# emmanuel-marty/zultra

Hardware: NVIDIA B200
Metric: input MB/s (zultra compression hot path, byte-identical to CPU zultra) (higher is better)
Workload: dtype u8

## Files before the change

### zultra_b200/csrc/zb_pipeline.h

```cpp
#ifndef ZB_PIPELINE_H
#define ZB_PIPELINE_H
#include "zb_rt.h"
#include <vector>
#include <algorithm>
#ifndef ZB_EMU
#include <cuda_pipeline.h>
#endif

#ifndef ZB_CG
#define ZB_CG 1024
#endif
#ifndef ZB_CP
#define ZB_CP 1024
#endif
#define ZB_CD 2048
#define ZB_WU 384
#define ZB_TOKI 256
#define ZB_NH 320
#define ZB_MAXSB 64
#define ZB_MAXNODES 64
#define ZB_MF_TILE_MAX 16384

struct ZbWinDesc {
   uint32_t in_off;
   uint32_t hist;
   uint32_t len;
   uint32_t stream;
   uint32_t last;
   uint32_t pad[3];
};

struct ZbNode {
   uint32_t win, depth;
   uint32_t ts, te;
   uint32_t ps, pe;
   uint32_t t0, nchk;
   uint32_t chk_base;
   int32_t total_cost;
   int32_t best_delta; uint32_t best_tok;
   uint32_t pad[4];
};

struct ZbSub {
   uint32_t win, idx_in_win;
   uint32_t ps, pe;
   uint32_t ts, te;
   int32_t is_dyn, static_cost, dynamic_cost;
   uint32_t dchunk_base, ndchunk;
   uint32_t pchunk_base, npchunk;
   int32_t mask, nl, no, ncl;
   int32_t hdr_bits;
   int32_t body_bits;
   int32_t stored;
   int32_t final_bit;
   uint64_t bit_off;
   int32_t ub_hit; int32_t pad;
};

struct ZbSubTabs {
   int lcnt[ZB_NLIT], ocnt[ZB_NOFF];
   int llen[ZB_NLIT], olen[ZB_NOFF];
   uint16_t lcode[ZB_NLIT], ocode[ZB_NOFF];
   int cllen[ZB_NCL]; uint16_t clcode[ZB_NCL];
   alignas(16) uint8_t cl[ZB_NLIT + ZB_NOFF]; int mask_cost[20];
   ZbCostTab cost;
};

struct ZbStreamOut {
   uint64_t out_word_off;
   uint64_t in_bits;
   uint64_t total_bits;
   uint32_t first_win, nwin;
   uint32_t err, pad;
};

ZB_HD void zb_tok_count(const uint8_t *T, uint32_t p, uint32_t len, uint32_t off, int *lc, int *oc, int sign) {
   if (len >= ZB_MIN_MATCH) { lc[zb_len_sym(len - ZB_MIN_MATCH)] += sign; oc[zb_off_sym(off)] += sign; }
   else lc[T[p]] += sign;
}

ZB_HD int zb_warmup_len(int WU, int reach) {
   const int margin = WU > ZB_MAX_MATCH ? WU - ZB_MAX_MATCH : 0;
   const int w = reach + margin;
   return w < WU ? w : WU;
}

template <class T> struct ZbBuf {
   T *p = 0; size_t cap = 0;
   void need(size_t n) { if (n > cap) { zb_dev_free(p); size_t c = n + n / 8 + 64; p = (T *)zb_dev_alloc(c * sizeof(T)); cap = p ? c : 0; } }
   void release() { zb_dev_free(p); p = 0; cap = 0; }
};

struct ZbHostBuf {
   uint8_t *p = 0; size_t cap = 0;
   void need(size_t n) { if (n > cap) { zb_host_free(p); size_t c = n + n / 8 + 4096; p = (uint8_t *)zb_host_alloc(c); cap = p ? c : 0; } }
   void release() { zb_host_free(p); p = 0; cap = 0; }
};

#ifndef ZB_EMU
#include <thread>
struct ZbStager {
   enum { LANES = 4, PIECE = 4 << 20 };
   uint8_t *buf = 0; cudaStream_t st[LANES]; cudaEvent_t ev[LANES][2]; bool ready = false;
   bool init() {
      if (ready) return true;
      if (cudaHostAlloc((void **)&buf, (size_t)LANES * 2 * PIECE, cudaHostAllocDefault) != cudaSuccess) { cudaGetLastError(); buf = 0; return false; }
      for (int l = 0; l < LANES; l++) { cudaStreamCreateWithFlags(&st[l], cudaStreamNonBlocking); cudaEventCreateWithFlags(&ev[l][0], cudaEventDisableTiming); cudaEventCreateWithFlags(&ev[l][1], cudaEventDisableTiming); }
      ready = true;
      return true;
   }
   void release() { if (!ready) return; for (int l = 0; l < LANES; l++) { cudaStreamDestroy(st[l]); cudaEventDestroy(ev[l][0]); cudaEventDestroy(ev[l][1]); } cudaFreeHost(buf); buf = 0; ready = false; }
   static bool pageable(const void *p) {
      cudaPointerAttributes a;
      if (cudaPointerGetAttributes(&a, p) != cudaSuccess) { cudaGetLastError(); return true; }
      return a.type == cudaMemoryTypeUnregistered;
   }
   bool copy(int dir, void *dev, void *host, size_t n, int device) {
      if (!init()) return false;
      bool ok[LANES];
      auto lane = [&](int l) {
         ok[l] = true;
         if (cudaSetDevice(device) != cudaSuccess) { ok[l] = false; return; }
         const size_t per = ((n + LANES - 1) / LANES + 255) & ~(size_t)255, lo = std::min(n, (size_t)l * per), hi = std::min(n, lo + per);
         uint8_t *b[2] = {buf + (size_t)(2 * l) * PIECE, buf + (size_t)(2 * l + 1) * PIECE};
         size_t pend_off[2] = {0, 0}, pend_len[2] = {0, 0};
         int k = 0;
         for (size_t off = lo; off < hi; off += PIECE, k ^= 1) {
            const size_t len = std::min((size_t)PIECE, hi - off);
            if (dir == 0) {
               if (cudaEventSynchronize(ev[l][k]) != cudaSuccess) ok[l] = false;
               memcpy(b[k], (const uint8_t *)host + off, len);
               if (cudaMemcpyAsync((uint8_t *)dev + off, b[k], len, cudaMemcpyHostToDevice, st[l]) != cudaSuccess) ok[l] = false;
               cudaEventRecord(ev[l][k], st[l]);
            } else {
               if (pend_len[k]) { if (cudaEventSynchronize(ev[l][k]) != cudaSuccess) ok[l] = false; memcpy((uint8_t *)host + pend_off[k], b[k], pend_len[k]); }
               if (cudaMemcpyAsync(b[k], (const uint8_t *)dev + off, len, cudaMemcpyDeviceToHost, st[l]) != cudaSuccess) ok[l] = false;
               cudaEventRecord(ev[l][k], st[l]);
               pend_off[k] = off; pend_len[k] = len;
            }
         }
         if (dir == 1) for (int q = 0; q < 2; q++, k ^= 1) if (pend_len[k]) { if (cudaEventSynchronize(ev[l][k]) != cudaSuccess) ok[l] = false; memcpy((uint8_t *)host + pend_off[k], b[k], pend_len[k]); pend_len[k] = 0; }
         if (cudaStreamSynchronize(st[l]) != cudaSuccess) ok[l] = false;
      };
      std::thread th[LANES - 1];
      for (int l = 1; l < LANES; l++) th[l - 1] = std::thread(lane, l);
      lane(0);
      for (int l = 1; l < LANES; l++) th[l - 1].join();
      for (int l = 0; l < LANES; l++) if (!ok[l]) { cudaGetLastError(); return false; }
      return true;
   }
};
#endif

struct ZbPipe {
   zb_stream_t st;
   ZbHostBuf hin, hout;
#ifndef ZB_EMU
   ZbStager stager;
   int device = 0;
#endif
   int nwin = 0, nstream = 0;
   uint32_t P = 0;
   std::vector<ZbWinDesc> h_win;
   std::vector<uint32_t> h_wbase;
   ZbBuf<ZbWinDesc> win; ZbBuf<uint32_t> wbase;
   ZbBuf<uint8_t> in;
   const uint8_t *in_ptr = 0;
   ZbBuf<uint64_t> keyA, keyB; ZbBuf<uint32_t> valA, valB, rank, sa, actA, actB, tmpA, tmpB, scratch;
   ZbBuf<uint32_t> sa_lcp;
   ZbBuf<uint32_t> counters;
   ZbBuf<ZbTileDesc> tiles, units, groups; ZbBuf<uint32_t> tile_iv, tile_pd, tile_cnt, tile_q, unit_words, unit_cnt, group_words, group_cnt, filt_seg;
   ZbBuf<zb_match_t> match; ZbBuf<uint16_t> glen, goff;
   ZbBuf<uint16_t> exitoff, exitc; ZbBuf<uint32_t> gentry, gtokcnt, gtokbase, tokpos, wtok;
   ZbBuf<uint32_t> wtokbase, wintbase; ZbBuf<int> ph;
   std::vector<uint32_t> h_gchunk_first; ZbBuf<uint32_t> gchunk_first, gchunk_win;
   ZbBuf<ZbNode> nodesA, nodesB; ZbBuf<int> nodehist; ZbBuf<uint16_t> chk_stat; ZbBuf<uint8_t> chk_flag; ZbBuf<int> chk_delta; ZbBuf<uint32_t> chk_node;
   ZbBuf<uint32_t> wsplit; ZbBuf<uint32_t> wnsplit, wsubcnt, wsubbase;
   ZbBuf<ZbSub> sub; ZbBuf<ZbSubTabs> tabs; ZbBuf<uint32_t> dchunk_sub, pchunk_sub;
   ZbBuf<zb_match_t> best; ZbBuf<int16_t> sig_true, sig_warm, sig_new; ZbBuf<uint8_t> dok; ZbBuf<uint32_t> dbad;
   ZbBuf<uint32_t> pentry, pbits, cand ; ZbBuf<uint16_t> dpfar;
   int cp = ZB_CP;
   ZbBuf<int> dreach;
   ZbBuf<uint32_t> out; ZbBuf<ZbStreamOut> sout;
   std::vector<ZbStreamOut> h_sout;
   int nsub = 0;
   bool sa_exact = false;
   int parse_cd = 0, parse_wu = ZB_WU;
   int mf_ts_min = ZB_TS_MIN, mf_ts_mul = ZB_TS_MUL;
   int stat_sa_rounds = 0, stat_redo = 0, stat_ub = 0, stat_tiles = 0;
   double t_stage[8];

   void release_all();
   void setup(const std::vector<ZbWinDesc> &wins, const uint8_t *h_in, size_t in_bytes, bool in_is_device);
   void stage_sa();
   void stage_match(uint32_t tile_main);
   void stage_greedy();
   void stage_split();
   void stage_parse();
   void stage_emit(const std::vector<ZbStreamOut> &streams) { stage_emit_prepare(); stage_emit_finish(streams); }
   void stage_emit_prepare();
   void stage_emit_finish(const std::vector<ZbStreamOut> &streams, uint32_t *ext_words = 0);
   void phase_maps(const std::vector<ZbStreamOut> &streams, unsigned long long *bits_out);
   std::vector<ZbStreamOut> plan;
   ZbBuf<uint32_t> ck_tab, ck_part; ZbBuf<uint64_t> ck_rng; bool ck_tab_ready = false;
   void stage_checksum(int kind, const std::vector<uint64_t> &range_off, const std::vector<uint64_t> &range_len, std::vector<uint32_t> &sums, uint32_t init_first);
};

ZB_HD int zb_find_win(const uint32_t *wbase, int nwin, uint32_t g) {
   int lo = 0, hi = nwin - 1;
   while (lo < hi) { int mid = (lo + hi + 1) >> 1; if (wbase[mid] <= g) lo = mid; else hi = mid - 1; }
   return lo;
}

inline void ZbPipe::setup(const std::vector<ZbWinDesc> &wins, const uint8_t *h_in, size_t in_bytes, bool in_is_device) {
   h_win = wins; nwin = (int)wins.size();
   h_wbase.assign(nwin + 1, 0);
   for (int w = 0; w < nwin; w++) h_wbase[w + 1] = h_wbase[w] + wins[w].len;
   P = h_wbase[nwin];
   win.need(nwin); wbase.need(nwin + 1); counters.need(64);
   if (!in_is_device) in.need(in_bytes + 16);
   if (zb_failed()) return;
   zb_h2d(st, win.p, h_win.data(), sizeof(ZbWinDesc) * nwin);
   zb_h2d(st, wbase.p, h_wbase.data(), 4 * (nwin + 1));
   if (in_is_device) in_ptr = h_in;
   else {
      if (h_in) {
#ifndef ZB_EMU
         if (in_bytes >= ((size_t)8 << 20) && ZbStager::pageable(h_in)) { zb_sync(st); if (!stager.copy(0, in.p, (void *)h_in, in_bytes, device)) zb_cuda_fail(cudaErrorUnknown); }
         else
#endif
         zb_h2d(st, in.p, h_in, in_bytes);
      }
      in_ptr = in.p;
   }
}

inline void ZbPipe::stage_sa() {
   const long n = P;
   keyA.need(n); keyB.need(n); valA.need(n); valB.need(n); rank.need(n); sa.need(n); actA.need(n); actB.need(n); tmpA.need(n + 1); tmpB.need(n + 1);
   sa_lcp.need(n);
   scratch.need(zb_sort_scratch_words(n) + zb_scan_scratch_words(n) + 64);
   if (zb_failed()) return;
   int wb = 0; while ((1L << wb) < nwin) wb++;
   int nbytes = (64 - wb) / 8; if (nbytes > 7) nbytes = 7;
   {
      static const int nb_env = getenv("ZULTRA_CUDA_SA_NBYTES") ? atoi(getenv("ZULTRA_CUDA_SA_NBYTES")) : 0;
      if (nb_env >= 3 && nb_env < nbytes) nbytes = nb_env;
   }
   const uint8_t *T = in_ptr; const ZbWinDesc *wd = win.p; const uint32_t *wbs = wbase.p; const int nw = nwin;
   uint64_t *kA = keyA.p; uint32_t *vA = valA.p;
   zb_tag("sa_keys");
   zb_launch(st, n, ZB_LAMBDA(long g) {
      int w = zb_find_win(wbs, nw, (uint32_t)g);
      uint32_t i = (uint32_t)g - wbs[w], len = wd[w].len;
      const uint8_t *t = T + wd[w].in_off;
      uint64_t k = 0;
      for (int b = 0; b < nbytes; b++) k = (k << 8) | (i + b < len ? t[i + b] : 0);
      kA[g] = ((uint64_t)w << (8 * nbytes)) | k;
      vA[g] = (uint32_t)g;
   }, 256);
   zb_sort_pairs(st, keyA.p, valA.p, keyB.p, valB.p, n, 0, 8 * nbytes + wb, scratch.p);
   uint32_t *head = tmpA.p, *grp = tmpB.p, *rk = rank.p, *SA = sa.p, *act = actA.p, *act2 = actB.p, *cnt = counters.p;
   zb_launch(st, n, ZB_LAMBDA(long j) { head[j] = (j == 0 || kA[j] != kA[j - 1]) ? (uint32_t)j : 0u; SA[j] = vA[j]; }, 256);
   zb_inclusive_max(st, head, grp, n, scratch.p);
   zb_launch(st, n, ZB_LAMBDA(long j) {
      const uint32_t gj = grp[j];
      rk[vA[j]] = gj;
      bool is_head = gj == (uint32_t)j;
      bool next_head = (j + 1 == n) || grp[j + 1] == (uint32_t)(j + 1);
      head[j] = (is_head && next_head) ? 0u : 1u;
   }, 256);
   zb_exclusive_sum(st, head, grp, n, cnt, scratch.p);
   zb_launch(st, n, ZB_LAMBDA(long j) { if (head[j]) act[grp[j]] = (uint32_t)j; }, 256);
   uint32_t m = 0;
   zb_d2h(st, &m, cnt, 4); zb_sync(st);
   int rank_bits = 1; while ((1L << rank_bits) < n) rank_bits++;
   uint64_t *kB = keyB.p; uint32_t *vB = valB.p;
   stat_sa_rounds = 0;
   uint32_t maxwin = 0;
   for (int w = 0; w < nwin; w++) maxwin = std::max(maxwin, h_win[w].len);
   int r2_bits = 1; while ((1L << r2_bits) < (long)maxwin + 512) r2_bits++;
   const bool packed_keys = !sa_exact;
   for (uint32_t h = (uint32_t)nbytes; m > 0 && (sa_exact || h < ZB_MAX_MATCH); h <<= 1) {
      stat_sa_rounds++;
      const long mm = m;
      zb_tag("sa_round_keys");
      if (packed_keys) {
         zb_launch(st, mm, ZB_LAMBDA(long a) {
            uint32_t j = act[a], g = SA[j];
            int w = zb_find_win(wbs, nw, g);
            uint32_t wend = wbs[w + 1];
            uint32_t r2;
            if ((uint64_t)g + h < wend) r2 = (rk[g + h] - wbs[w]) + 512u;
            else r2 = wend - g;
            kA[a] = ((uint64_t)rk[g] << r2_bits) | r2;
            vA[a] = g;
         }, 256);
         zb_sort_pairs(st, keyA.p, valA.p, keyB.p, valB.p, mm, 0, r2_bits + rank_bits, scratch.p);
      } else {
      zb_launch(st, mm, ZB_LAMBDA(long a) {
         uint32_t j = act[a], g = SA[j];
         int w = zb_find_win(wbs, nw, g);
         uint32_t wend = wbs[w + 1];
         uint32_t r2;
         if ((uint64_t)g + h < wend) r2 = (rk[g + h] - wbs[w]) + (1u << 22);
         else r2 = wend - g;
         kA[a] = ((uint64_t)rk[g] << 32) | r2;
         vA[a] = g;
      }, 256);
      zb_sort_pairs(st, keyA.p, valA.p, keyB.p, valB.p, mm, 0, 23, scratch.p);
      zb_sort_pairs(st, keyA.p, valA.p, keyB.p, valB.p, mm, 32, 32 + rank_bits, scratch.p);
      }
      zb_launch(st, mm, ZB_LAMBDA(long a) { head[a] = (a == 0 || kA[a] != kA[a - 1]) ? (uint32_t)a : 0u; SA[act[a]] = vA[a]; }, 256);
      zb_inclusive_max(st, head, grp, mm, scratch.p);
      zb_launch(st, mm, ZB_LAMBDA(long a) {
         const uint32_t ga = grp[a];
         rk[vA[a]] = act[ga];
         bool is_head = ga == (uint32_t)a;
         bool next_head = (a + 1 == mm) || grp[a + 1] == (uint32_t)(a + 1);
         head[a] = (is_head && next_head) ? 0u : 1u;
      }, 256);
      zb_exclusive_sum(st, head, (uint32_t *)kB, mm, cnt, scratch.p);
      {
         const uint32_t *dst = (const uint32_t *)kB;
         zb_launch(st, mm, ZB_LAMBDA(long a) { if (head[a]) act2[dst[a]] = act[a]; }, 256);
      }
      zb_d2h(st, &m, cnt, 4); zb_sync(st);
      std::swap(act, act2);
      (void)vB;
      if (h > (1u << 23)) break;
   }
   uint32_t *out = sa_lcp.p;
   zb_tag("lcp_pack");
   zb_launch(st, n, ZB_LAMBDA(long j) {
      uint32_t g = SA[j];
      int w = zb_find_win(wbs, nw, (uint32_t)j);
      uint32_t base = wbs[w], len = wd[w].len;
      uint32_t i = g - base;
      uint32_t l = 0;
      if ((uint32_t)j != base) {
         uint32_t q = SA[j - 1] - base;
         const uint8_t *t = T + wd[w].in_off;
         uint32_t lim = len - (i > q ? i : q);
         if (lim > ZB_MAX_MATCH) lim = ZB_MAX_MATCH;
#ifdef __CUDA_ARCH__
         if (wd[w].in_off + (i < q ? i : q) >= 4) {
            while (l + 8 <= lim) {
               const uintptr_t a = (uintptr_t)(t + i + l), b = (uintptr_t)(t + q + l);
               const uint32_t *pa = (const uint32_t *)(a & ~(uintptr_t)3), *pb = (const uint32_t *)(b & ~(uintptr_t)3);
               const uint32_t x = __funnelshift_r(pa[0], pa[1], (uint32_t)(a & 3) << 3) ^ __funnelshift_r(pb[0], pb[1], (uint32_t)(b & 3) << 3);
               if (x) { l += (uint32_t)(__ffs((int)x) - 1) >> 3; lim = l; break; }
               l += 4;
            }
         }
#endif
         while (l < lim && t[i + l] == t[q + l]) l++;
         if (l < ZB_MIN_MATCH) l = 0;
      }
      out[j] = i | (l << ZB_POS_BITS);
   }, 256);
}

#ifndef ZB_EMU
#define ZB_MF_THREADS 1024
__global__ void __launch_bounds__(ZB_MF_THREADS) zb_mf_scan_k(const ZbTileDesc *td, int first, const uint32_t *unit_words, const uint32_t *unit_cnt, uint32_t *queues, size_t qstride,
                                                              size_t stride, uint32_t *qcnt, zb_match_t *mt, uint16_t *gl, uint16_t *go, const uint32_t *wbs, uint32_t tile_main,
                                                              int ts_min, int ts_mul) {
   extern __shared__ __align__(16) uint32_t zb_smw[];
   __shared__ uint32_t next_m, nq, wcnt[32], wtail[32];
   const int k = blockIdx.x;
   const ZbTileDesc t = td[first + k];
   const uint32_t nlook = t.m0 - t.lo, nmain = t.hi - t.m0;
   uint32_t *words = zb_smw + 1;
   uint16_t *rom = (uint16_t *)(zb_smw + stride + 2);
   uint32_t *queue = queues + (size_t)k * qstride;
   int n = 0;
   {
      const uint32_t *src = unit_words + t.src_base;
      const uint32_t nsrc = unit_cnt[t.src_cnt_idx];
      const uint32_t lo_rel = t.lo - t.src_lo, span = t.hi - t.lo;
      const int lane = threadIdx.x & 31, warp = threadIdx.x >> 5;
      const uint32_t lt = (1u << lane) - 1u;
      uint32_t count = 0, carry = 0x1ffu;
      uint32_t wn[4];
#pragma unroll
      for (int j = 0; j < 4; j++) { const uint32_t r = (uint32_t)j * ZB_MF_THREADS + threadIdx.x; wn[j] = r < nsrc ? __ldg(src + r) : 0u; }
      for (uint32_t g0 = 0; g0 < nsrc; g0 += 4 * ZB_MF_THREADS) {
      uint32_t wc[4];
#pragma unroll
      for (int j = 0; j < 4; j++) { wc[j] = wn[j]; const uint32_t r = g0 + (uint32_t)(4 + j) * ZB_MF_THREADS + threadIdx.x; wn[j] = r < nsrc ? __ldg(src + r) : 0u; }
#pragma unroll
      for (int j = 0; j < 4; j++) {
         const uint32_t r0 = g0 + (uint32_t)j * ZB_MF_THREADS;
         if (r0 >= nsrc) break;
         const uint32_t r = r0 + threadIdx.x;
         const bool valid = r < nsrc;
         const uint32_t w = wc[j];
         const uint32_t pos = (w & ZB_POS_MASK) - lo_rel;
         uint32_t v = valid ? ((w >> ZB_POS_BITS) & 0x1ffu) : 0x1ffu;
         const bool keep = valid && pos < span;
         const uint32_t kmask = __ballot_sync(0xffffffffu, keep);
         const uint32_t below = kmask & lt;
         const int start = below ? (32 - __clz((int)below)) : 0;
#pragma unroll
         for (int d = 1; d < 32; d <<= 1) {
            const uint32_t o = __shfl_up_sync(0xffffffffu, v, d);
            if (lane >= start + d) v = min(v, o);
         }
         const uint32_t v31 = __shfl_sync(0xffffffffu, v, 31);
         if (lane == 0) { wcnt[warp] = __popc(kmask); wtail[warp] = ((kmask >> 31) ? 0x1ffu : v31) | (kmask ? 0x10000u : 0u); }
         __syncthreads();
         const uint32_t cx = wcnt[lane], tx = wtail[lane];
         uint32_t inc = cx;
#pragma unroll
         for (int d = 1; d < 32; d <<= 1) { const uint32_t o = __shfl_up_sync(0xffffffffu, inc, d); if (lane >= d) inc += o; }
         const uint32_t prefix = __shfl_sync(0xffffffffu, inc - cx, warp), total = __shfl_sync(0xffffffffu, inc, 31);
         const uint32_t hasmask = __ballot_sync(0xffffffffu, (tx >> 16) & 1u);
         const uint32_t hb = hasmask & ((1u << warp) - 1u);
         const int lo_u = hb ? 31 - __clz((int)hb) : 0;
         uint32_t cin = __reduce_min_sync(0xffffffffu, (lane >= lo_u && lane < warp) ? (tx & 0xffffu) : 0x1ffu);
         if (!hb) cin = min(cin, carry);
         const int lo_2 = hasmask ? 31 - __clz((int)hasmask) : 0;
         uint32_t cnew = __reduce_min_sync(0xffffffffu, lane >= lo_2 ? (tx & 0xffffu) : 0x1ffu);
         if (!hasmask) cnew = min(cnew, carry);
         if (start == 0) v = min(v, cin);
         if (keep) {
            const uint32_t at = count + prefix + __popc(below);
            words[at] = pos | (v << ZB_POS_BITS);
            if (pos >= nlook) rom[pos - nlook] = (uint16_t)at;
         }
         count += total; carry = cnew;
         __syncthreads();
      }
      }
      n = (int)count;
   }
   if (threadIdx.x == 0) { next_m = 0; nq = 0; zb_smw[0] = 0; words[n] = 0; }
   __syncthreads();
   const uint32_t gbase = wbs[t.win];
   const int lane = threadIdx.x & 31;
   bool busy = false, drained = false, moved = false;
   uint32_t m = 0, lL = 0, lR = 0, lvl = 0, maxlen = 0, rec0 = 0, rec1 = 0;
   int i = 0, L = 0, R = 0, best = -1, nm = 0, steps = 0, gap = 0, thr = 0;
   uint32_t *dst = 0;
#define ZB_MF_EMIT(v_) do { uint32_t v__ = (v_); if ((v__ & 0xffffu) > maxlen) v__ = (v__ & 0xffff0000u) | maxlen; \
      if (nm == 0) rec0 = v__; else if (nm == 1) rec1 = v__; else dst[nm] = v__; nm++; } while (0)
   for (;;) {
      {
         const uint32_t need = __ballot_sync(0xffffffffu, !busy && !drained);
         if (need) {
            uint32_t base = 0;
            if (lane == __ffs((int)need) - 1) base = atomicAdd(&next_m, (uint32_t)__popc(need));
            base = __shfl_sync(0xffffffffu, base, __ffs((int)need) - 1);
            if (!busy && !drained) {
               m = base + (uint32_t)__popc(need & ((1u << lane) - 1u));
               if (m >= nmain) drained = true;
               else {
                  busy = true;
                  const int r = (int)rom[m];
                  i = (int)(nlook + m);
                  L = r - 1; R = r + 1;
                  lL = words[r] >> ZB_POS_BITS;
                  lR = words[R] >> ZB_POS_BITS;
                  best = (i > ZB_MAX_OFFSET ? i - ZB_MAX_OFFSET : 0) - 1;
                  nm = 0; lvl = 0; moved = false; steps = 0; rec0 = 0; rec1 = 0;
                  gap = i - 1 - best; thr = 0;
                  maxlen = t.wlen - (t.m0 + m);
                  dst = (uint32_t *)(mt + ((size_t)(gbase + t.m0 + m) << 3));
               }
            }
         }
      }
      if (__all_sync(0xffffffffu, !busy)) break;
      bool fin = false;
      if (busy) {
#pragma unroll 1
         for (int step = 0; step < 8; step++) {
            const uint32_t l = lL > lR ? lL : lR;
            if (l < lvl && moved) {
               ZB_MF_EMIT(lvl | ((uint32_t)(i - best) << 16));
               moved = false;
               if (nm == ZB_NMATCH) { fin = true; break; }
            }
            if (l < ZB_MIN_MATCH) { fin = true; break; }
            if (steps >= ts_min && gap <= thr) {
               const uint32_t at = atomicAdd(&nq, 1u);
               if (nm == 1) dst[0] = rec0; else if (nm >= 2) *(uint2 *)dst = make_uint2(rec0, rec1);
               queue[3 * at] = m | ((uint32_t)nm << 14) | ((moved ? 1u : 0u) << 18) | (lvl << 19);
               queue[3 * at + 1] = l | ((uint32_t)(i - 1 - best) << 9);
               queue[3 * at + 2] = rec0;
               busy = false;
               break;
            }
            lvl = l; steps++; thr += ts_mul;
            const bool goL = lL > lR || (lL == lR && (steps & 1));
            const int at = goL ? L : R;
            const uint32_t w = words[at], w2 = words[at + 1];
            const uint32_t wl = (goL ? w : w2) >> ZB_POS_BITS;
            L -= goL ? 1 : 0; R += goL ? 0 : 1;
            const uint32_t side = goL ? lL : lR;
            const uint32_t nl = wl < side ? wl : side;
            lL = goL ? nl : lL; lR = goL ? lR : nl;
            const int p = (int)(w & ZB_POS_MASK);
            if (p < i && p > best) {
               best = p; moved = true;
               if (best == i - 1) { ZB_MF_EMIT(lvl | (1u << 16)); fin = true; break; }
               gap = i - 1 - best;
            }
         }
      }
      if (fin) {
         *(uint2 *)dst = make_uint2(rec0, nm >= 2 ? rec1 : 0u);
         if (nm <= 2) { *(uint2 *)(dst + 2) = make_uint2(0u, 0u); *(uint4 *)(dst + 4) = make_uint4(0u, 0u, 0u, 0u); }
         else for (int z = nm; z < ZB_NMATCH; z++) dst[z] = 0u;
         const uint32_t p = t.m0 + m;
         const uint32_t l0 = rec0 & 0xffffu;
         gl[gbase + p] = l0 >= ZB_MIN_MATCH ? (uint16_t)l0 : (uint16_t)1;
         go[gbase + p] = l0 >= ZB_MIN_MATCH ? (uint16_t)(rec0 >> 16) : (uint16_t)0;
         busy = false;
      }
   }
#undef ZB_MF_EMIT
   __syncthreads();
   if (threadIdx.x == 0) qcnt[k] = nq;
}

#define ZB_MT_THREADS 512
__global__ void __launch_bounds__(ZB_MT_THREADS) zb_mf_text_k(const ZbTileDesc *td, int first, const uint32_t *lists, size_t stride, const uint32_t *qcnt,
                                                              zb_match_t *mt, uint16_t *gl, uint16_t *go, const uint32_t *wbs, const ZbWinDesc *wd, const uint8_t *T) {
   extern __shared__ __align__(16) uint32_t zb_smw[];
   __shared__ uint32_t next_q;
   __shared__ __align__(8) uint64_t txt_bar;
   const int k = blockIdx.x;
   const uint32_t nq = qcnt[k];
   if (nq == 0) return;
   const ZbTileDesc t = td[first + k];
   const uint32_t nlook = t.m0 - t.lo;
   const uint32_t *queue = lists + (size_t)k * stride;
   const uint8_t *tsrc = T + wd[t.win].in_off + t.lo;
   const uint32_t delta = (uint32_t)((uintptr_t)tsrc & 15u);
   uint8_t *txt = (uint8_t *)zb_smw;
   {
      uint32_t ntxt = t.hi - t.lo + ZB_MAX_MATCH;
      if (ntxt > t.wlen - t.lo) ntxt = t.wlen - t.lo;
      uint32_t head = (16u - delta) & 15u; if (head > ntxt) head = ntxt;
      const uint32_t bulk = (ntxt - head) & ~15u;
      const uint32_t bar = (uint32_t)__cvta_generic_to_shared(&txt_bar);
      if (threadIdx.x == 0) {
         asm volatile("mbarrier.init.shared::cta.b64 [%0], 1;" :: "r"(bar));
         asm volatile("fence.proxy.async.shared::cta;" ::: "memory");
         if (bulk) {
            asm volatile("mbarrier.arrive.expect_tx.shared::cta.b64 _, [%0], %1;" :: "r"(bar), "r"(bulk) : "memory");
            asm volatile("cp.async.bulk.shared::cluster.global.mbarrier::complete_tx::bytes [%0], [%1], %2, [%3];"
                         :: "r"((uint32_t)__cvta_generic_to_shared(txt + delta + head)), "l"(tsrc + head), "r"(bulk), "r"(bar) : "memory");
         }
      }
      for (uint32_t e = threadIdx.x; e < head; e += blockDim.x) txt[delta + e] = tsrc[e];
      for (uint32_t e = head + bulk + threadIdx.x; e < ntxt; e += blockDim.x) txt[delta + e] = tsrc[e];
      __syncthreads();
      if (bulk) {
         uint32_t ok = 0;
         while (!ok) asm volatile("{ .reg .pred p; mbarrier.try_wait.parity.shared::cta.b64 p, [%1], 0; selp.u32 %0, 1, 0, p; }" : "=r"(ok) : "r"(bar) : "memory");
      }
   }
   if (threadIdx.x == 0) next_q = 0;
   __syncthreads();
   const uint32_t gbase = wbs[t.win];
   const int lane = threadIdx.x & 31;
   for (;;) {
      uint32_t e0 = 0;
      if (lane == 0) e0 = atomicAdd(&next_q, 32u);
      e0 = __shfl_sync(0xffffffffu, e0, 0);
      if (e0 >= nq) break;
// ... 2436 lines not shown
```

Baseline: 1461.

## Fuse SA group detection and locally resolve small buckets with extra key bytes

Replaces the head-mark, inclusive-max scan and rank kernels after the initial suffix-array radix sort with a single kernel. Each element finds its group head by exponential plus binary search. Groups smaller than 32 are refined in place by comparing the next 8 bytes of text plus a length tiebreak, so singletons settle without prefix-doubling rounds. This removes one scan and two launches and cuts the number of active suffixes entering the doubling loop. In exchange it adds per-thread serial searches and quadratic work within small groups, and exact ranks depend on the tie-break logic being correct.

Result: faster. 1506, median of 6 (+3.1%).

```diff
diff --git a/zultra_b200/csrc/zb_pipeline.h b/zultra_b200/csrc/zb_pipeline.h
--- a/zultra_b200/csrc/zb_pipeline.h
+++ b/zultra_b200/csrc/zb_pipeline.h
@@ -235,6 +235,26 @@
    }
 }
 
+#define ZB_SA_LOCAL 32
+
+ZB_HD void zb_sa_key(const uint8_t *t, uint32_t i, uint32_t len, uint32_t d, uint64_t &w, uint32_t &tl) {
+   const uint32_t rem = len - i;
+   tl = rem < d + 9 ? rem : d + 9;
+#ifdef __CUDA_ARCH__
+   if ((uint64_t)i + d + 12 <= len) {
+      const uintptr_t a = (uintptr_t)(t + i + d);
+      const uint32_t *pa = (const uint32_t *)(a & ~(uintptr_t)3);
+      const uint32_t sh = (uint32_t)(a & 3) << 3;
+      const uint32_t x0 = __funnelshift_r(pa[0], pa[1], sh), x1 = __funnelshift_r(pa[1], pa[2], sh);
+      w = ((uint64_t)__byte_perm(x0, 0, 0x0123) << 32) | __byte_perm(x1, 0, 0x0123);
+      return;
+   }
+#endif
+   uint64_t x = 0;
+   for (uint32_t b = 0; b < 8; b++) x = (x << 8) | ((uint64_t)i + d + b < len ? t[i + d + b] : 0u);
+   w = x;
+}
+
 inline void ZbPipe::stage_sa() {
    const long n = P;
    keyA.need(n); keyB.need(n); valA.need(n); valB.need(n); rank.need(n); sa.need(n); actA.need(n); actB.need(n); tmpA.need(n + 1); tmpB.need(n + 1);
@@ -261,14 +281,35 @@
    }, 256);
    zb_sort_pairs(st, keyA.p, valA.p, keyB.p, valB.p, n, 0, 8 * nbytes + wb, scratch.p);
    uint32_t *head = tmpA.p, *grp = tmpB.p, *rk = rank.p, *SA = sa.p, *act = actA.p, *act2 = actB.p, *cnt = counters.p;
-   zb_launch(st, n, ZB_LAMBDA(long j) { head[j] = (j == 0 || kA[j] != kA[j - 1]) ? (uint32_t)j : 0u; SA[j] = vA[j]; }, 256);
-   zb_inclusive_max(st, head, grp, n, scratch.p);
-   zb_launch(st, n, ZB_LAMBDA(long j) {
-      const uint32_t gj = grp[j];
-      rk[vA[j]] = gj;
-      bool is_head = gj == (uint32_t)j;
-      bool next_head = (j + 1 == n) || grp[j + 1] == (uint32_t)(j + 1);
-      head[j] = (is_head && next_head) ? 0u : 1u;
+   const int kbits = 8 * nbytes;
+   zb_tag("sa_group");
+   zb_launch(st, n, ZB_LAMBDA(long jl) {
+      const uint32_t j = (uint32_t)jl;
+      const uint64_t key = kA[j];
+      uint32_t gh = j, step = 1;
+      while (gh >= step && kA[gh - step] == key) { gh -= step; step <<= 1; }
+      long lo = gh >= step ? (long)(gh - step) : -1L;
+      while ((long)gh - lo > 1) { const uint32_t mid = (uint32_t)((lo + (long)gh) >> 1); if (kA[mid] == key) gh = mid; else lo = mid; }
+      const uint32_t g = vA[j];
+      if ((long)gh + ZB_SA_LOCAL < n && kA[gh + ZB_SA_LOCAL] == key) { SA[j] = g; rk[g] = gh; head[j] = 1u; return; }
+      uint32_t ge = j + 1;
+      while ((long)ge < n && kA[ge] == key) ge++;
+      if (ge - gh == 1) { SA[j] = g; rk[g] = j; head[j] = 0u; return; }
+      const int w = (int)(key >> kbits);
+      const uint32_t base = wbs[w], len = wd[w].len;
+      const uint8_t *t = T + wd[w].in_off;
+      uint64_t kw; uint32_t kt;
+      zb_sa_key(t, g - base, len, (uint32_t)nbytes, kw, kt);
+      uint32_t less = 0, eq_before = 0, eq = 0;
+      for (uint32_t y = gh; y < ge; y++) {
+         if (y == j) continue;
+         uint64_t yw; uint32_t yt;
+         zb_sa_key(t, vA[y] - base, len, (uint32_t)nbytes, yw, yt);
+         if (yw < kw || (yw == kw && yt < kt)) less++;
+         else if (yw == kw && yt == kt) { eq++; if (y < j) eq_before++; }
+      }
+      const uint32_t p = gh + less + eq_before;
+      SA[p] = g; rk[g] = gh + less; head[p] = eq ? 1u : 0u;
    }, 256);
    zb_exclusive_sum(st, head, grp, n, cnt, scratch.p);
    zb_launch(st, n, ZB_LAMBDA(long j) { if (head[j]) act[grp[j]] = (uint32_t)j; }, 256);
```
